# mcdiarmid/waveforms

Measured on AMD Instinct MI355X. Metric: SOQPSK-TG Msym/s mod+Viterbi-detect @8sps, higher is better.
Workload: dtype f64; 1 GPU; SOQPSK-TG 1e+07 symbols @8 sps, modulate + AWGN + PT matched filter + 4-state Viterbi detect (BASELINE configs[1]); waveform=soqpsk, sps=8, prbs=PN23, noise=Philox4x32-10 + Box-Muller (device), fuse=175, streams=1, detector_warmup_rows=16, detector_form=lanes (one chunk per lane), parallelism=independent trial blocks x1

## Files before the change

waveforms_amd/_hip.py:

```python
from __future__ import annotations

import ctypes
import threading
from ctypes import POINTER, c_char_p, c_double, c_int, c_int64, c_uint64, c_void_p
from pathlib import Path

import numpy as np

import os

_LIB_PATH = Path(os.environ.get("WF_HIP_LIBRARY") or Path(__file__).resolve().parent / "csrc" / "libwfhip.so")

WF_ERR_VALUE, WF_ERR_KEY, WF_ERR_HIP, WF_ERR_DEVICE, WF_ERR_NOMEM = -1, -2, -3, -4, -5
WF_CPM_STATE_BYTES, WF_CPM_STREAM_STATE_BYTES = 16384, 20480
(WF_OPT_CPM_FORM, WF_OPT_CPM_CHUNK_CALLS, WF_OPT_DET_REPAIR, WF_OPT_DET_FINAL_VERIFY, WF_OPT_ITERATION_SERVER,
 WF_OPT_MCB_TAIL_PERMILLE, WF_OPT_PIPE_RESERVE_CUS, WF_OPT_CPM_SAMPLES_MIN_CALLS, WF_OPT_SOFT_CHUNK_CALLS,
 WF_OPT_CPM_SOFT_CHUNK_CALLS) = range(10)

_P = c_void_p
SIGNATURES = {
    "wf_version": (c_char_p, []),
    "wf_last_error_string": (c_char_p, []),
    "wf_ctx_create": (c_int, [c_int, POINTER(c_void_p)]),
    "wf_ctx_destroy": (c_int, [_P]),
# ... 133 lines not shown
        ("warmup", c_int), ("fuse", c_int), ("event_slot", c_int), ("d_mf_factor", c_void_p),
    ]


_lib = None
_lock = threading.RLock()
_ctxs: dict[int, int] = {}


def lib() -> ctypes.CDLL:
    global _lib
    if _lib is None:
        with _lock:
            if _lib is None:
                if not _LIB_PATH.exists():
                    raise RuntimeError(
                        f"{_LIB_PATH} is missing - build it with `python -m waveforms_amd.csrc.build` "
                        "(there is no CPU fallback)")
                import torch

                handle = ctypes.CDLL(str(_LIB_PATH))
                for name, (res, args) in SIGNATURES.items():
                    fn = getattr(handle, name)
                    fn.restype, fn.argtypes = res, args
                _lib = handle
    return _lib


def torch():
    import torch as _t

    return _t


def require_device() -> int:
    t = torch()
    if not t.cuda.is_available():
        raise RuntimeError("waveforms_amd needs a HIP device (MI355X); none is visible and there is "
                           "no CPU fallback")
    return t.cuda.current_device()


def check(rc: int) -> None:
    if rc == 0:
        return
    msg = lib().wf_last_error_string().decode(errors="replace")
    if rc == WF_ERR_VALUE:
        raise ValueError(msg)
    if rc == WF_ERR_KEY:
        raise KeyError(msg)
    raise RuntimeError(f"libwfhip error {rc}: {msg}")


default_options: dict[int, int] = {}


def set_option(handle, key: int, value: int) -> None:
    check(lib().wf_ctx_set_option(handle, int(key), int(value)))


def get_option(handle, key: int) -> int:
    v = c_int64(0)
    check(lib().wf_ctx_get_option(handle, int(key), ctypes.byref(v)))
    return int(v.value)


def set_default_option(key: int, value: int) -> None:
    with _lock:
        if int(value) == 0:
            default_options.pop(int(key), None)
        else:
            default_options[int(key)] = int(value)
        for handle in _ctxs.values():
            set_option(handle, key, value)


def apply_option_args(pairs) -> None:
    for kv in pairs or []:
        key, _, val = str(kv).partition("=")
        set_default_option(globals()["WF_OPT_" + key.strip().upper()], int(val))


def ctx() -> int:
    dev = require_device()
    if dev not in _ctxs:
        with _lock:
            if dev not in _ctxs:
                out = c_void_p()
                check(lib().wf_ctx_create(dev, ctypes.byref(out)))
                for k, v in default_options.items():
                    set_option(out.value, k, v)
                if not _ctxs:
                    import atexit

                    atexit.register(_destroy_default_contexts)
                _ctxs[dev] = out.value
    return _ctxs[dev]


def _destroy_default_contexts() -> None:
    for handle in list(_ctxs.values()):
        try:
            if _lib is not None:
                _lib.wf_ctx_retire(handle)
        except Exception:
            pass


def new_ctx() -> int:
    out = c_void_p()
    check(lib().wf_ctx_create(require_device(), ctypes.byref(out)))
    for k, v in default_options.items():
        set_option(out.value, k, v)
    return out.value


def free_ctx(handle) -> None:
    if handle and _lib is not None:
        try:
            _lib.wf_ctx_destroy(handle)
        except Exception:
            pass


def stream() -> int:
    return torch().cuda.current_stream().cuda_stream


def device_check() -> None:
    check(lib().wf_ctx_check(ctx(), stream()))


_NP2T = {"uint8": "uint8", "int8": "int8", "float64": "float64", "int64": "int64", "int32": "int32", "float32": "float32"}
# ... 35 lines not shown
```

waveforms_amd/csrc/wf_common.h:

```cpp
#pragma once
#include <hip/hip_runtime.h>
#include <stdint.h>

#include <atomic>
#include <map>
#include <mutex>
#include <vector>
#include <string>

#include "../../include/wfhip.h"

#define WF_WAVE 64

void wf_set_error(const char *fmt, ...);

#define WF_HIP(call)                                                                     \
    do {                                                                                 \
        hipError_t e_ = (call);                                                          \
        if (e_ != hipSuccess) {                                                          \
            wf_set_error("%s failed: %s (%s:%d)", #call, hipGetErrorString(e_), __FILE__, \
                         __LINE__);                                                      \
            return WF_ERR_HIP;                                                           \
        }                                                                                \
    } while (0)

#define WF_REQUIRE(cond, ...)          \
    do {                               \
        if (!(cond)) {                 \
            wf_set_error(__VA_ARGS__); \
            return WF_ERR_VALUE;       \
        }                              \
    } while (0)

#define WF_LAUNCH_CHECK() WF_HIP(hipGetLastError())

enum { WF_FAULT_SCAN_TIMEOUT = 1u, WF_FAULT_LIVE_TABLE = 2u };

struct wf_lfsr_tables {
    uint64_t host[64][64];
    uint64_t *dev = nullptr;
    uint64_t f_even = 0, f_odd = 0, f_m2 = 0, f_m1 = 0;
    bool f_ready = false;
};

struct wf_ctx {
    int device = 0;
    int cus = 256;
    int64_t opt[WF_OPT_COUNT] = {0};
    uint64_t *d_scan = nullptr;
    size_t scan_words = 0;
    unsigned *d_fault = nullptr;
    unsigned *h_fault = nullptr;
    uint8_t *d_tables = nullptr;
    uint8_t h_tables_cache[2048] = {0};
    int tables_cached = 0;
    hipEvent_t tables_event = nullptr;
    hipStream_t tables_stream = nullptr;
    bool tables_pending = false;
    uint64_t *d_fsm_scratch = nullptr;
    size_t fsm_scratch_words = 0;
    int *h_small = nullptr;
    int *d_small = nullptr;
    std::map<uint64_t, wf_lfsr_tables *> lfsr;
    double *d_mod_scratch = nullptr;
    size_t mod_scratch_words = 0;
    double *d_vit_edge = nullptr;
    size_t vit_edge_words = 0;
    unsigned long long *d_vit_unmerged = nullptr;
    hipEvent_t *events = nullptr;
    void *pipe_stream = nullptr;
    void *pipe_stream2 = nullptr;
    void *pipe_pro = nullptr, *pipe_main = nullptr;
    hipEvent_t pipe_call = nullptr, pipe_pro_done = nullptr;
    hipEvent_t pipe_front = nullptr, pipe_done[2] = {nullptr, nullptr};
    bool pipe_done_valid[2] = {false, false};
    int pipe_set = 0;
    std::map<uint64_t, uint32_t> promises;
    std::mutex promises_lock;
    double *h_iter = nullptr;
    double *d_iter = nullptr;
    void *h_mailbox = nullptr;
    void *d_mailbox = nullptr;
    void *iter_stream = nullptr;
    const void *iter_last_state = nullptr;
    std::atomic_flag iter_lock = ATOMIC_FLAG_INIT;
    bool iter_closing = false;
};

static inline hipStream_t wf_stream(void *s) { return reinterpret_cast<hipStream_t>(s); }

int wf_ctx_reserve_scan(wf_ctx *ctx, size_t words);
int wf_ctx_reserve_fsm(wf_ctx *ctx, size_t words);
int wf_ctx_reserve_mod(wf_ctx *ctx, size_t words);
int wf_iter_server_stop(wf_ctx *ctx);
int wf_ctx_reserve_vit(wf_ctx *ctx, size_t words);

struct lfsr_emit_args;
int wf_lfsr_generate_dyn(wf_ctx *ctx, int degree, uint64_t mask, uint64_t state, uint64_t skip,
                         const uint64_t *d_dyn_skip, uint8_t *d_bits, int64_t n, uint64_t *h_state_out, void *stream,
                         const struct lfsr_emit_args *emit = nullptr);
int wf_lfsr_generate_map(wf_ctx *ctx, int degree, uint64_t mask, uint64_t state, uint64_t skip, uint8_t *d_bits, int64_t nbits,
                         int map_kind, int8_t *d_symbols, void *stream);
int wf_soqpsk_prbs_encode(wf_ctx *ctx, int degree, uint64_t mask, uint64_t state, uint64_t skip, const uint8_t *h_next,
                          const int8_t *h_out, uint8_t *d_bits, int64_t n, int8_t *d_symbols, void *stream, void *mid_event = nullptr);
int wf_awgn_mf_bank_dyn(wf_ctx *ctx, const double *d_signal_ri, int64_t nsamp, double rot_re, double rot_im,
                        double sigma, uint64_t seed, uint64_t stream_id, uint64_t first_index,
                        const uint64_t *d_dyn_index, const double *d_taps_ri, int nfilt, int ntaps, int64_t first,
                        int step, int64_t ncols, double *d_out_ri, void *stream, int pack_par0 = -1);
int wf_viterbi4_detect_packed(wf_ctx *ctx, const double *d_rows4, int64_t ncalls, int differential, int warmup,
                              uint8_t *d_bits, int8_t *d_syms, double *d_state, void *stream);
int wf_cpm_modulate_window(wf_ctx *ctx, const int8_t *d_symbols, int64_t sym_origin, int64_t nloc, int64_t nsym_total,
                           const double *d_h, int nh, const double *d_pulse, int ntaps, int sps, double phi0,
                           int64_t tile_lo, int64_t ntiles, double *d_out_ri, int64_t out_origin,
                           const uint64_t *d_q_in, uint64_t *d_q_out, int64_t q_out_tile, void *stream);
struct wf_mcb_opts {
    const double *pam_factor = nullptr;
    bool cpm_paired = false;
    int runs_hint = 0;
    int scratch_slot = -1;
};
int wf_mod_chan_bank_packed(wf_ctx *ctx, const int8_t *d_symbols, int64_t nsym, const double *d_h, int nh,
                            const double *d_pulse, int ntaps, int sps, double phi0, const double *d_mf_taps, double rot_re,
                            double rot_im, double sigma, uint64_t seed, uint64_t stream_id, uint64_t first_index,
                            int64_t first, int64_t ncols, int pack_par0, double *d_rows4, void *stream, int mf_ntaps = 0,
                            const wf_mcb_opts *opts = nullptr, int stage = 3);
int wf_mod_chan_bank_window(wf_ctx *ctx, const int8_t *d_symbols, int64_t sym_origin, int64_t nloc, int64_t nsym_total,
// ... 404 lines not shown
```

waveforms_amd/csrc/wf_ctx.hip:

```cpp
#include <stdarg.h>
#include <stdio.h>

#include "wf_common.h"

static thread_local char g_err[512] = "";

void wf_set_error(const char *fmt, ...)
{
    va_list ap;
    va_start(ap, fmt);
    vsnprintf(g_err, sizeof(g_err), fmt, ap);
    va_end(ap);
}

extern "C" const char *wf_version(void) { return "waveforms-amd 0.1.0 (gfx950)"; }
extern "C" const char *wf_last_error_string(void) { return g_err; }

extern "C" int wf_ctx_create(int device, wf_ctx **out)
{
    WF_REQUIRE(out != nullptr, "wf_ctx_create: out is NULL");
    int ndev = 0;
    WF_HIP(hipGetDeviceCount(&ndev));
    WF_REQUIRE(device >= 0 && device < ndev, "wf_ctx_create: device %d of %d", device, ndev);
    WF_HIP(hipSetDevice(device));
    wf_ctx *c = new wf_ctx();
    c->device = device;
    (void)hipDeviceGetAttribute(&c->cus, hipDeviceAttributeMultiprocessorCount, device);
    if (c->cus < 1) c->cus = 256;
    WF_HIP(hipMalloc(&c->d_fault, 64));
    WF_HIP(hipMemset(c->d_fault, 0, 64));
    WF_HIP(hipHostMalloc(&c->h_fault, 64, hipHostMallocDefault));
    WF_HIP(hipMalloc(&c->d_tables, 4096));
    WF_HIP(hipMalloc(&c->d_vit_unmerged, 4 * sizeof(unsigned long long)));
    WF_HIP(hipMemset(c->d_vit_unmerged, 0, 4 * sizeof(unsigned long long)));
    WF_HIP(hipMalloc(&c->d_small, 256));
    WF_HIP(hipHostMalloc(&c->h_small, 256, hipHostMallocDefault));
    *out = c;
    int rc = wf_ctx_reserve_scan(c, 1 << 16);
    if (rc) return rc;
    return wf_ctx_reserve_fsm(c, 1 << 16);
}

extern "C" int wf_ctx_destroy(wf_ctx *c)
{
    if (!c) return WF_OK;
    (void)hipSetDevice(c->device);
    (void)wf_iter_server_stop(c);
    (void)hipDeviceSynchronize();
    for (auto &kv : c->lfsr) {
        if (kv.second->dev) (void)hipFree(kv.second->dev);
        delete kv.second;
    }
    if (c->events) {
        for (int k = 0; k < WF_LINK_EVENT_SLOTS * (WF_LINK_STAGES + 1); ++k) (void)hipEventDestroy(c->events[k]);
        delete[] c->events;
    }
    if (c->pipe_front) (void)hipEventDestroy(c->pipe_front);
    for (int k = 0; k < 2; ++k)
        if (c->pipe_done[k]) (void)hipEventDestroy(c->pipe_done[k]);
    if (c->pipe_stream) (void)hipStreamDestroy(static_cast<hipStream_t>(c->pipe_stream));
    if (c->pipe_stream2) (void)hipStreamDestroy(static_cast<hipStream_t>(c->pipe_stream2));
    if (c->pipe_pro) (void)hipStreamDestroy(static_cast<hipStream_t>(c->pipe_pro));
    if (c->pipe_main) (void)hipStreamDestroy(static_cast<hipStream_t>(c->pipe_main));
    if (c->pipe_call) (void)hipEventDestroy(c->pipe_call);
    if (c->pipe_pro_done) (void)hipEventDestroy(c->pipe_pro_done);
    if (c->d_scan) (void)hipFree(c->d_scan);
    if (c->d_fsm_scratch) (void)hipFree(c->d_fsm_scratch);
    if (c->d_mod_scratch) (void)hipFree(c->d_mod_scratch);
    if (c->d_vit_edge) (void)hipFree(c->d_vit_edge);
    if (c->d_vit_unmerged) (void)hipFree(c->d_vit_unmerged);
    if (c->d_fault) (void)hipFree(c->d_fault);
    if (c->h_fault) (void)hipHostFree(c->h_fault);
    if (c->d_tables) (void)hipFree(c->d_tables);
    if (c->tables_event) (void)hipEventDestroy(c->tables_event);
    if (c->d_small) (void)hipFree(c->d_small);
    if (c->h_small) (void)hipHostFree(c->h_small);
    if (c->h_iter) (void)hipHostFree(c->h_iter);
    if (c->iter_stream) (void)hipStreamDestroy(static_cast<hipStream_t>(c->iter_stream));
    if (c->h_mailbox) (void)hipHostFree(c->h_mailbox);
    delete c;
    return WF_OK;
}

extern "C" int wf_ctx_retire(wf_ctx *c)
{
    if (!c) return WF_OK;
    (void)hipSetDevice(c->device);
    (void)wf_iter_server_stop(c);
    if (c->pipe_stream) (void)hipStreamSynchronize(static_cast<hipStream_t>(c->pipe_stream));
    if (c->pipe_stream2) (void)hipStreamSynchronize(static_cast<hipStream_t>(c->pipe_stream2));
    if (c->pipe_pro) (void)hipStreamSynchronize(static_cast<hipStream_t>(c->pipe_pro));
    if (c->pipe_main) (void)hipStreamSynchronize(static_cast<hipStream_t>(c->pipe_main));
    return WF_OK;
}

int wf_link_join_internal(wf_ctx *c, void *stream)
{
    if (!c) return WF_OK;
    for (int k = 0; k < 2; ++k)
        if (c->pipe_done_valid[k]) WF_HIP(hipStreamWaitEvent(wf_stream(stream), c->pipe_done[k], 0));
    return WF_OK;
}

extern "C" int wf_link_join(wf_ctx *c, void *stream)
{
    WF_REQUIRE(c != nullptr, "wf_link_join: ctx is NULL");
    return wf_link_join_internal(c, stream);
}

extern "C" int wf_ctx_set_option(wf_ctx *c, int key, int64_t value)
{
    WF_REQUIRE(c != nullptr, "wf_ctx_set_option: ctx is NULL");
    WF_REQUIRE(key >= 0 && key < WF_OPT_COUNT, "wf_ctx_set_option: unknown option %d", key);
    bool ok = true;
    switch (key) {
    case WF_OPT_CPM_FORM: ok = value >= 0 && value <= 2; break;
    case WF_OPT_CPM_CHUNK_CALLS: ok = value >= 0 && value <= 8192; break;
    case WF_OPT_DET_REPAIR: case WF_OPT_DET_FINAL_VERIFY: case WF_OPT_ITERATION_SERVER: ok = value == 0 || value == 1; break;
// ... 143 lines not shown
```

waveforms_amd/csrc/wf_link.h:

```cpp
#pragma once
#include "wf_common.h"

static inline int64_t round_up(int64_t v, int64_t a) { return (v + a - 1) / a * a; }

static inline int link_pipe_open(wf_ctx *ctx, const char *fn, int64_t set_bytes, int64_t workspace_bytes, bool second)
{
    WF_REQUIRE(2 * set_bytes <= workspace_bytes, "%s: fuse bit 5 needs two sets of intermediates (%lld bytes)", fn, (long long)(2 * set_bytes));
    WF_HIP(hipSetDevice(ctx->device));
    hipStream_t ps;
    if (!ctx->pipe_stream) {
        WF_HIP(hipStreamCreateWithFlags(&ps, hipStreamNonBlocking));
        ctx->pipe_stream = ps;
        WF_HIP(hipEventCreateWithFlags(&ctx->pipe_front, hipEventDisableTiming));
        for (int k = 0; k < 2; ++k) WF_HIP(hipEventCreateWithFlags(&ctx->pipe_done[k], hipEventDisableTiming));
    }
    if (second && !ctx->pipe_stream2) {
        WF_HIP(hipStreamCreateWithFlags(&ps, hipStreamNonBlocking));
        ctx->pipe_stream2 = ps;
    }
    return WF_OK;
}

static inline int link_pipe_select(wf_ctx *ctx, int64_t set_bytes, char *&w, void *waiter)
{
    w += (int64_t)ctx->pipe_set * set_bytes;
    if (ctx->pipe_done_valid[ctx->pipe_set]) WF_HIP(hipStreamWaitEvent(wf_stream(waiter), ctx->pipe_done[ctx->pipe_set], 0));
    return WF_OK;
}

static inline int link_pipe_close(wf_ctx *ctx, void *back)
{
    WF_HIP(hipEventRecord(ctx->pipe_done[ctx->pipe_set], wf_stream(back)));
    ctx->pipe_done_valid[ctx->pipe_set] = true;
    ctx->pipe_set ^= 1;
    return WF_OK;
}

static inline int link_stage_events(wf_ctx *ctx, const char *fn, int event_slot, hipEvent_t *&ev)
{
    ev = nullptr;
    if (event_slot < 0) return WF_OK;
    WF_REQUIRE(event_slot < WF_LINK_EVENT_SLOTS, "%s: event_slot %d", fn, event_slot);
    if (!ctx->events) {
        ctx->events = new hipEvent_t[WF_LINK_EVENT_SLOTS * (WF_LINK_STAGES + 1)];
        for (int k = 0; k < WF_LINK_EVENT_SLOTS * (WF_LINK_STAGES + 1); ++k) WF_HIP(hipEventCreate(&ctx->events[k]));
    }
    ev = ctx->events + event_slot * (WF_LINK_STAGES + 1);
    return WF_OK;
}

static inline int mark(hipEvent_t *ev, int k, void *stream)
{
    if (ev) WF_HIP(hipEventRecord(ev[k], wf_stream(stream)));
    return WF_OK;
}

struct link_chunk_window {
    int64_t k_lo, ncols, ws, nloc, tile_lo, tile_hi, ntiles, q_out_tile;
};

static inline link_chunk_window link_chunk_window_of(int64_t B, int64_t c, int64_t halo, int64_t N, int64_t ncalls_total, int64_t spt, int64_t ntiles_total)
{
    link_chunk_window W;
    W.k_lo = c * B;
    const int64_t k_hi = W.k_lo + B < ncalls_total ? W.k_lo + B : ncalls_total;
    W.ncols = k_hi > W.k_lo ? k_hi - W.k_lo : 0;
    W.ws = c * B - halo > 0 ? c * B - halo : 0;
    const int64_t we = (c + 1) * B + halo < N ? (c + 1) * B + halo : N;
    W.nloc = we > W.ws ? we - W.ws : 0;
    W.tile_lo = spt > 0 && c * B / spt - 1 > 0 ? c * B / spt - 1 : 0;
    W.tile_hi = spt > 0 ? (c + 1) * B / spt + 1 : 0;
    if (W.tile_hi > ntiles_total) W.tile_hi = ntiles_total;
    W.ntiles = W.tile_hi > W.tile_lo ? W.tile_hi - W.tile_lo : 0;
    const int64_t next_tile_lo = spt > 0 ? (c + 1) * B / spt - 1 : 0;
    W.q_out_tile = (next_tile_lo >= W.tile_lo && next_tile_lo < W.tile_hi) ? next_tile_lo - W.tile_lo : -1;
    return W;
}
// ... 19 lines not shown
```

waveforms_amd/csrc/wf_pipeline.hip:

```cpp
#include "wf_link.h"

__global__ void time_axis_kernel(int64_t n, double step, double *__restrict__ out)
{
    const int64_t stride = (int64_t)gridDim.x * blockDim.x;
    for (int64_t k = (int64_t)blockIdx.x * blockDim.x + threadIdx.x; k < n; k += stride)
        out[k] = (double)k * step;
}

extern "C" int wf_time_axis_f64(wf_ctx *ctx, int64_t n, double step, double *d_out, void *stream)
{
    WF_REQUIRE(ctx && n >= 0, "wf_time_axis_f64: bad argument");
    if (n == 0) return WF_OK;
    WF_REQUIRE(d_out != nullptr, "wf_time_axis_f64: NULL output");
    WF_HIP(hipSetDevice(ctx->device));
    hipLaunchKernelGGL(time_axis_kernel, dim3(wf_grid_for(n, 256, 4096)), dim3(256), 0, wf_stream(stream), n,
                       step, d_out);
    WF_LAUNCH_CHECK();
    return WF_OK;
}

struct link_layout {
    int64_t nsym, npts, ncols, first;
    size_t off_bits, off_syms, off_freq, off_sig, off_mf, off_dbits, off_dsyms, total;
};
// ... 59 lines not shown
}
static int link_check_factor(wf_ctx *ctx, const wf_link_config *cfg, void *stream)
{
    if (!cfg->d_mf_factor || cfg->mf_ntaps == cfg->sps + 1 || cfg->mf_nfilt != 3 || cfg->mf_ntaps < 1) return WF_OK;
    const int nt = cfg->mf_ntaps;
    const void *ptrs[2] = {cfg->d_mf_taps, cfg->d_mf_factor};
    const size_t nb[2] = {(size_t)3 * nt * 16, (size_t)(2 * nt + 12) * 8};
    return wf_promise_verified(ctx, 2, ptrs, nb, 2, stream, link_factor_matches, &nt,
                               "wf_link_config.d_mf_factor does not reproduce d_mf_taps (taps[s] != sum_k G[s][k] b_k to 1e-12)");
}

extern "C" int64_t wf_link_workspace_bytes(const wf_link_config *cfg)
{
    if (!cfg || cfg->nsym < 1 || cfg->sps < 1) return -1;
    const int64_t one = (int64_t)make_layout(cfg->nsym, cfg->sps, cfg->ntaps, cfg->mf_nfilt, 2, cfg->timing_offset).total;
    return link_pipelined(cfg) ? 2 * round_up(one, 256) : one;
}

static hipStream_t link_masked_stream(const wf_ctx *ctx, int reserve)
{
    hipStream_t s = nullptr;
    if (reserve > 0 && reserve < ctx->cus) {
        const int words = (ctx->cus + 31) / 32;
        std::vector<uint32_t> mask((size_t)words, 0u);
        for (int cu = reserve; cu < ctx->cus; ++cu) mask[(size_t)(cu / 32)] |= 1u << (cu % 32);
        if (hipExtStreamCreateWithCUMask(&s, (uint32_t)words, mask.data()) == hipSuccess) return s;
        (void)hipGetLastError();
        s = nullptr;
    }
    if (hipStreamCreateWithFlags(&s, hipStreamDefault) != hipSuccess) return nullptr;
    return s;
}

extern "C" int wf_link_run(wf_ctx *ctx, const wf_link_config *cfg, void *d_workspace, int64_t workspace_bytes,
                           int64_t *d_counts, int64_t *h_compared, void *stream)
{
    WF_REQUIRE(ctx && cfg && d_workspace && d_counts, "wf_link_run: NULL argument");
    WF_REQUIRE(cfg->nsym >= 1 && cfg->sps >= 1 && cfg->mf_nfilt == 3, "wf_link_run: bad configuration");
    WF_REQUIRE((reinterpret_cast<uintptr_t>(d_workspace) & 255) == 0, "wf_link_run: workspace must be 256-byte aligned");
    const int length = 2;
    const link_layout L = make_layout(cfg->nsym, cfg->sps, cfg->ntaps, cfg->mf_nfilt, length, cfg->timing_offset);
    WF_REQUIRE((int64_t)L.total <= workspace_bytes, "wf_link_run: workspace too small (%lld < %lld)",
               (long long)workspace_bytes, (long long)L.total);
    WF_REQUIRE(L.npts >= cfg->mf_ntaps, "wf_link_run: burst shorter than the matched filter");
    char *w = static_cast<char *>(d_workspace);
    const bool piped = link_pipelined(cfg) && L.ncols > 0;
    void *s_pro = stream, *s_main = stream;
    bool ahead = false;
    int slot = -1, rc;
    if (piped) {
        const int64_t set_bytes = round_up((int64_t)L.total, 256);
        if ((rc = link_pipe_open(ctx, "wf_link_run", set_bytes, workspace_bytes, false))) return rc;
        const int64_t rsv = ctx->opt[WF_OPT_PIPE_RESERVE_CUS];
        ahead = rsv != 0;
        if (ahead) {
            if (!ctx->pipe_pro) {
                hipStream_t sp;
                WF_HIP(hipStreamCreateWithFlags(&sp, hipStreamDefault));
                ctx->pipe_pro = sp;
                ctx->pipe_main = link_masked_stream(ctx, rsv < 0 ? 0 : (int)rsv);
                WF_REQUIRE(ctx->pipe_main != nullptr, "wf_link_run: could not create the front end's stream");
                WF_HIP(hipEventCreateWithFlags(&ctx->pipe_call, hipEventDisableTiming));
                WF_HIP(hipEventCreateWithFlags(&ctx->pipe_pro_done, hipEventDisableTiming));
            }
            s_pro = ctx->pipe_pro;
            s_main = ctx->pipe_main;
            slot = ctx->pipe_set;
            if (stream) {
                WF_HIP(hipEventRecord(ctx->pipe_call, wf_stream(stream)));
                WF_HIP(hipStreamWaitEvent(wf_stream(s_pro), ctx->pipe_call, 0));
            }
        }
        if ((rc = link_pipe_select(ctx, set_bytes, w, s_pro))) return rc;
    } else if ((rc = wf_link_join_internal(ctx, stream))) {
        return rc;
    }
    uint8_t *bits = reinterpret_cast<uint8_t *>(w + L.off_bits);
    int8_t *syms = reinterpret_cast<int8_t *>(w + L.off_syms);
    double *freq = reinterpret_cast<double *>(w + L.off_freq);
    double *sig = reinterpret_cast<double *>(w + L.off_sig);
    double *mf = reinterpret_cast<double *>(w + L.off_mf);
    uint8_t *dbits = reinterpret_cast<uint8_t *>(w + L.off_dbits);
    int8_t *dsyms = reinterpret_cast<int8_t *>(w + L.off_dsyms);

    const soqpsk_trellis_tables T = soqpsk_trellis(cfg->differential);
    hipEvent_t *ev;
    if ((rc = link_stage_events(ctx, "wf_link_run", cfg->event_slot, ev))) return rc;
    if ((rc = mark(ev, 0, s_pro))) return rc;
    rc = (cfg->fuse & 16) ? 1 : wf_soqpsk_prbs_encode(ctx, cfg->degree, cfg->mask, cfg->state, cfg->skip, &T.next[0][0][0], &T.outp[0][0][0], bits,
                                                       cfg->nsym, syms, s_pro, ev ? (void *)ev[1] : nullptr);
    if (rc < 0) return rc;
    if (rc == 1) {
        if ((rc = wf_lfsr_generate(ctx, cfg->degree, cfg->mask, cfg->state, cfg->skip, bits, cfg->nsym, nullptr, s_pro))) return rc;
        if ((rc = mark(ev, 1, s_pro))) return rc;
        if ((rc = wf_fsm_encode(ctx, &T.next[0][0][0], &T.outp[0][0][0], 2, 4, 1, bits, cfg->nsym, 0, 0, syms, nullptr, s_pro))) return rc;
    }
    if (!ahead && (rc = mark(ev, 2, s_pro))) return rc;
    bool fused_all = false;
    if (link_one_kernel(cfg) && L.ncols > 0) {
        wf_mcb_opts mo;
        mo.pam_factor = cfg->d_mf_factor;
        mo.scratch_slot = slot;
        if ((rc = link_check_factor(ctx, cfg, stream))) return rc;
        for (int stage = ahead ? 1 : 3; stage <= (ahead ? 2 : 3); ++stage) {
            if (ahead && stage == 2) {
                if ((rc = mark(ev, 2, s_pro))) return rc;
                WF_HIP(hipEventRecord(ctx->pipe_pro_done, wf_stream(s_pro)));
                WF_HIP(hipStreamWaitEvent(wf_stream(s_main), ctx->pipe_pro_done, 0));
                if ((rc = mark(ev, 3, s_main))) return rc;
            }
            rc = wf_mod_chan_bank_packed(ctx, syms, cfg->nsym, cfg->d_h, 1, cfg->d_pulse, cfg->ntaps, cfg->sps, M_PI / 4, cfg->d_mf_taps,
                                         cos(-M_PI / 4), sin(-M_PI / 4), cfg->sigma, cfg->seed, cfg->stream_id, 0, L.first, L.ncols, 0,
                                         mf, stage == 1 ? s_pro : s_main, cfg->mf_ntaps, &mo, stage);
            if (rc < 0) return rc;
            WF_REQUIRE(rc == 0, "wf_link_run: internal: the one-kernel front end refused a configuration wf_mod_chan_bank_applies accepted");
        }
        fused_all = true;
    }
    if (fused_all) {
        if (!ahead && (rc = mark(ev, 3, s_main))) return rc;
        if ((rc = mark(ev, 4, s_main)) || (rc = mark(ev, 5, s_main))) return rc;
        void *back = stream;
        if (piped) {
            back = ctx->pipe_stream;
            WF_HIP(hipEventRecord(ctx->pipe_front, wf_stream(s_main)));
            WF_HIP(hipStreamWaitEvent(wf_stream(back), ctx->pipe_front, 0));
        }
        if ((rc = mark(ev, 6, back))) return rc;
        rc = wf_viterbi4_detect_packed(ctx, mf, L.ncols, cfg->differential, link_warmup(cfg), dbits, dsyms, nullptr, back);
        if (rc) return rc;
        if ((rc = mark(ev, 7, back))) return rc;
        int64_t m_ = L.ncols - length;
        if (m_ > cfg->nsym) m_ = cfg->nsym;
        if (m_ < 0) m_ = 0;
        if ((rc = wf_count_errors(ctx, dsyms + length, syms, dbits + length, bits, m_, d_counts, back))) return rc;
        if ((rc = mark(ev, 8, back))) return rc;
        if (piped && (rc = link_pipe_close(ctx, back))) return rc;
        if (h_compared) *h_compared = m_;
        return WF_OK;
    }
    bool fused_mod = false;
    if (cfg->fuse & 1) {
        rc = wf_cpm_modulate_c128(ctx, syms, cfg->nsym, cfg->d_h, 1, cfg->d_pulse, cfg->ntaps, cfg->sps, M_PI / 4, sig, stream);
        if (rc < 0) return rc;
        fused_mod = rc == 0;
    }
    if (fused_mod) {
        if ((rc = mark(ev, 3, stream))) return rc;
    } else {
        if ((rc = wf_upsample_fir_f64(ctx, syms, cfg->nsym, cfg->d_h, 1, cfg->d_pulse, cfg->ntaps, cfg->sps, freq, stream))) return rc;
        if ((rc = mark(ev, 3, stream))) return rc;
        if ((rc = wf_phase_cexp_f64(ctx, freq, L.npts, cfg->sps, M_PI / 4, 0.0, sig, nullptr, stream))) return rc;
    }
    if ((rc = mark(ev, 4, stream))) return rc;
    const double rot_re = cos(-M_PI / 4), rot_im = sin(-M_PI / 4);
    const bool fused_chan = (cfg->fuse & 2) && L.ncols > 0;
    if (!fused_chan)
        if ((rc = wf_awgn_c128(ctx, sig, L.npts, rot_re, rot_im, cfg->sigma, cfg->seed, cfg->stream_id, 0, sig, stream))) return rc;
    if ((rc = mark(ev, 5, stream))) return rc;
    int64_t m = L.ncols - length;
    if (m > cfg->nsym) m = cfg->nsym;
    if (m < 0) m = 0;
    const bool packed = fused_chan && link_packed_rows8(cfg);
    if (L.ncols > 0) {
        if (packed)
            rc = wf_awgn_mf_bank_dyn(ctx, sig, L.npts, rot_re, rot_im, cfg->sigma, cfg->seed, cfg->stream_id, 0, nullptr,
                                     cfg->d_mf_taps, cfg->mf_nfilt, cfg->mf_ntaps, L.first, cfg->sps, L.ncols, mf, stream, 0);
        else if (fused_chan)
            rc = wf_awgn_mf_bank_c128(ctx, sig, L.npts, rot_re, rot_im, cfg->sigma, cfg->seed, cfg->stream_id, 0,
                                      cfg->d_mf_taps, cfg->mf_nfilt, cfg->mf_ntaps, L.first, cfg->sps, L.ncols, mf, stream);
        else
            rc = wf_mf_bank_c128(ctx, sig, L.npts, cfg->d_mf_taps, cfg->mf_nfilt, cfg->mf_ntaps, L.first, cfg->sps,
                                 L.ncols, mf, stream);
        if (rc) return rc;
        if ((rc = mark(ev, 6, stream))) return rc;
        if (packed)
            rc = wf_viterbi4_detect_packed(ctx, mf, L.ncols, cfg->differential, link_warmup(cfg), dbits, dsyms, nullptr, stream);
        else
            rc = wf_viterbi4_detect(ctx, mf, L.ncols, cfg->differential, link_warmup(cfg), dbits, dsyms, nullptr, stream);
// ... 251 lines not shown
```

waveforms_amd/csrc/wf_viterbi.hip:

```cpp
#include <stddef.h>
#include <stdlib.h>
#include <string.h>

#include <time.h>

#include "wf_viterbi4.h"

#define VIT_THREADS 256
#define VIT_DEFAULT_WARMUP 31
#define VIT_MAX_LEN 64

template <int COL>
__device__ __forceinline__ void vit_acs(const double m[4], const vit_comp &q, double out[4], uint64_t second[4])
{
    double fa[4], fb[4];
    if (COL == 0) {
        fa[0] = m[0] - q.i1; fb[0] = m[2] + q.a;
        fa[1] = m[1] - q.r1; fb[1] = m[3] + q.b;
        fa[2] = m[0] - q.b;  fb[2] = m[2] + q.r1;
        fa[3] = m[1] - q.a;  fb[3] = m[3] + q.i1;
    } else {
        fa[0] = m[0] - q.i1; fb[0] = m[1] - q.b;
        fa[1] = m[0] - q.a;  fb[1] = m[1] - q.r1;
        fa[2] = m[2] + q.r1; fb[2] = m[3] + q.a;
// ... 20 lines not shown
{
    constexpr int PREV = COL ^ 1;
    const vit_comp now = vit_components<COL, PACKED>(zrow);
    const double mn = fmin(fmin(L.m0[0], L.m0[1]), fmin(L.m0[2], L.m0[3]));
    const double carried[4] = {L.m0[0] - mn, L.m0[1] - mn, L.m0[2] - mn, L.m0[3] - mn};
    double ma[4], mb[4];
    uint64_t n0[4], n1[4];
    vit_acs<PREV>(carried, L.prev, ma, n0);
    vit_acs<COL>(ma, now, mb, n1);
    const uint64_t c01 = __builtin_amdgcn_ballot_w64(mb[1] < mb[0]), c23 = __builtin_amdgcn_ballot_w64(mb[3] < mb[2]);
    const double v01 = fmin(mb[0], mb[1]), v23 = fmin(mb[2], mb[3]);
    const uint64_t s1b1 = __builtin_amdgcn_ballot_w64(v23 < v01);
    const uint64_t s1b0 = vit_mux(s1b1, c23, c01);
    const uint64_t w1 = vit_mux(s1b1, vit_mux(c23, n1[3], n1[2]), vit_mux(c01, n1[1], n1[0]));
    const uint64_t e0b0 = COL == 0 ? s1b0 : w1;
    const uint64_t e0b1 = COL == 0 ? w1 : s1b1;
    const uint64_t w0 = vit_mux(e0b1, vit_mux(e0b0, n0[3], n0[2]), vit_mux(e0b0, n0[1], n0[0]));
    const uint64_t st0b0 = PREV == 0 ? e0b0 : w0;
    const uint64_t st0b1 = PREV == 0 ? w0 : e0b1;
    const uint64_t b0 = PREV == 0 ? e0b1 : e0b0, b1 = st0b0, b2 = st0b1;
    const uint64_t bit_m = b0 ^ (diff ? (PREV == 0 ? st0b1 : st0b0) : 0ull);
    const uint64_t x02 = b0 ^ b2, x01 = b0 ^ b1, x12 = b1 ^ b2;
    const uint64_t cd0_m = PREV == 0 ? ~x02 : ~x01;
    const uint64_t cd1_m = PREV == 0 ? (x02 & ~x12) : (x01 & ~x02);
    bit = __builtin_amdgcn_inverse_ballot_w64(bit_m);
    cd0 = __builtin_amdgcn_inverse_ballot_w64(cd0_m);
    cd1 = __builtin_amdgcn_inverse_ballot_w64(cd1_m);
#pragma unroll
    for (int s = 0; s < 4; ++s) L.m0[s] = ma[s];
    L.prev = now;
}

template <int COL, bool PACKED>
__device__ __forceinline__ void vit_step(vit_lane &L, const double2 *__restrict__ zrow, bool prime, int diff,
                                         int64_t k, int64_t a, int64_t ncalls, uint64_t *__restrict__ dec)
{
    if (prime) {
        L.prev = vit_components<COL, PACKED>(zrow);
        return;
    }
    bool bit, cd0, cd1;
    vit_step_core<COL, PACKED>(L, zrow, diff, bit, cd0, cd1);
    if (k >= a) {
        const int c = (int)(k - a) & 15;
        L.wb |= (bit ? 1u : 0u) << c;
        L.ws |= ((cd0 ? 1u : 0u) | (cd1 ? 2u : 0u)) << (2 * c);
        if (c == 15 || k + 1 == ncalls) {
            dec[(int)(k - a) >> 4] = (uint64_t)L.wb | ((uint64_t)L.ws << 32);
            L.wb = L.ws = 0;
        }
    }
}

__device__ __forceinline__ uint64_t vit_spread_bits8(uint32_t x)
{
    const uint64_t t = ((uint64_t)(x & 0xFF) * 0x0101010101010101ull) & 0x8040201008040201ull;
    return ((t + 0x7F7F7F7F7F7F7F7Full) >> 7) & 0x0101010101010101ull;
}

__device__ __forceinline__ uint64_t vit_spread_syms8(uint32_t x)
{
    uint64_t t = ((uint64_t)(x & 0xFFFF) | ((uint64_t)(x & 0xFFFF) << 24)) & 0x000000FF000000FFull;
    t = (t | (t << 12)) & 0x000F000F000F000Full;
    t = (t | (t << 6)) & 0x0303030303030303ull;
    const uint64_t v = t << 1;
    return ((v & 0x7F7F7F7F7F7F7F7Full) + 0x7E7E7E7E7E7E7E7Eull) ^ ((v ^ 0xFEFEFEFEFEFEFEFEull) & 0x8080808080808080ull);
}

__device__ __forceinline__ void vit_flush(const uint64_t *__restrict__ dec, int ch, int64_t a, int64_t ncalls,
                                          uint8_t *__restrict__ bits, int8_t *__restrict__ syms)
{
    for (int gq = 0; gq < ch / 16; ++gq) {
        const int64_t k0 = a + 16 * gq;
        if (k0 >= ncalls) break;
        const uint64_t w = dec[gq];
        const uint32_t wb = (uint32_t)w, ws = (uint32_t)(w >> 32);
        const uint64_t b_lo = vit_spread_bits8(wb), b_hi = vit_spread_bits8(wb >> 8);
        const uint64_t s_lo = vit_spread_syms8(ws), s_hi = vit_spread_syms8(ws >> 16);
        if (k0 + 16 <= ncalls) {
            *reinterpret_cast<ulonglong2 *>(bits + k0) = make_ulonglong2(b_lo, b_hi);
            *reinterpret_cast<ulonglong2 *>(syms + k0) = make_ulonglong2(s_lo, s_hi);
        } else {
            for (int q = 0; k0 + q < ncalls; ++q) {
                bits[k0 + q] = (uint8_t)(((q < 8 ? b_lo : b_hi) >> (8 * (q & 7))) & 0xFF);
                syms[k0 + q] = (int8_t)(((q < 8 ? s_lo : s_hi) >> (8 * (q & 7))) & 0xFF);
            }
        }
    }
}

__device__ __forceinline__ void vit_save_start(vit_lane &L)
{
#pragma unroll
    for (int s4 = 0; s4 < 4; ++s4) L.ms[s4] = L.m0[s4];
}

__device__ __forceinline__ vit_comp vit_comp_from_inc(const double *inc, int col)
{
    vit_comp c;
    c.i1 = inc[7];
    if (col == 0) { c.a = inc[4]; c.r1 = inc[5]; c.b = inc[6]; }
    else { c.r1 = inc[4]; c.b = inc[5]; c.a = inc[6]; }
    return c;
}

__device__ __forceinline__ void vit_comp_to_inc(const vit_comp &c, int col, double *inc)
{
    if (col == 0) {
        inc[0] = -c.i1; inc[1] = -c.b; inc[2] = -c.r1; inc[3] = -c.a;
        inc[4] = c.a;   inc[5] = c.r1; inc[6] = c.b;   inc[7] = c.i1;
    } else {
        inc[0] = -c.i1; inc[1] = -c.a; inc[2] = -c.b;  inc[3] = -c.r1;
        inc[4] = c.r1;  inc[5] = c.b;  inc[6] = c.a;   inc[7] = c.i1;
    }
}

#define VIT_S 4
#ifndef VIT_DEPTH
#define VIT_DEPTH 3
#endif
#define VIT_PIECES_RW(RW) ((RW) * VIT_S)
#define VIT_PIECES (3 * VIT_S)
#define VIT_LANE_SLOTS (VIT_PIECES + 1)

__device__ __forceinline__ double2 vit_ld16(const double2 *p)
{
    typedef double v2d __attribute__((ext_vector_type(2)));
    const v2d v = __builtin_nontemporal_load(reinterpret_cast<const v2d *>(p));
    return make_double2(v.x, v.y);
}

template <int PAR0, bool PACKED>
__device__ __forceinline__ void viterbi_batch_body(const double *__restrict__ mf, int64_t ncalls, int CH, int diff, int warmup,
                                                   uint8_t *__restrict__ bits, int8_t *__restrict__ syms,
                                                   double *__restrict__ state, int64_t i0, double2 (*s_rows)[WF_WAVE * VIT_LANE_SLOTS],
                                                   uint64_t *__restrict__ s_dec, double *__restrict__ edge)
{
    constexpr int RW = PACKED ? 2 : 3;
    constexpr int NP = VIT_PIECES_RW(RW);
    constexpr int LS = NP + 1;
    const int lane = threadIdx.x & 63, wave = threadIdx.x >> 6;
    const int64_t g0 = ((int64_t)blockIdx.x * (VIT_THREADS / WF_WAVE) + wave) * WF_WAVE;
    const int64_t a = (g0 + lane) * CH;
    const bool live = a < ncalls;
    const int nsteps = warmup + 1 + CH;
    const int nbatch = (nsteps + VIT_S - 1) / VIT_S;
    const double2 *rows = reinterpret_cast<const double2 *>(mf);
    double2 *tile = s_rows[wave];
    uint64_t *dec = s_dec + (wave * WF_WAVE + lane) * (CH / 16 + 1);
// ... 2 lines not shown
#pragma unroll
    for (int u = 0; u < NP; ++u) {
        const int p = u * WF_WAVE + lane;
        const int sg = p / NP;
        sgw[u] = (sg << 8) | (p - sg * NP);
    }
    const int64_t g0u = __builtin_amdgcn_readfirstlane((int)(g0 >> 6)) * (int64_t)WF_WAVE;
    auto fetch = [&](int b, double2 dst[NP]) __attribute__((always_inline)) {
        const int64_t rb = g0u * CH - warmup - 1 + (int64_t)b * VIT_S;
        const double2 *basep = rows + RW * rb;
        if (rb >= 0 && rb + (int64_t)(WF_WAVE - 1) * CH + VIT_S <= ncalls) {
#pragma unroll
            for (int u = 0; u < NP; ++u) dst[u] = vit_ld16(basep + RW * CH * (sgw[u] >> 8) + (sgw[u] & 255));
        } else {
            const int64_t lo64 = -rb, hi64 = ncalls - 1 - rb;
            const int lo = lo64 < -(1 << 30) ? -(1 << 30) : (lo64 > (1 << 30) ? (1 << 30) : (int)lo64);
            const int hi = hi64 < -(1 << 30) ? -(1 << 30) : (hi64 > (1 << 30) ? (1 << 30) : (int)hi64);
#pragma unroll
            for (int u = 0; u < NP; ++u) {
                const int sg = sgw[u] >> 8, wi = sgw[u] & 255;
                const int rrel = sg * CH + wi / RW;
                const int rc = min(max(rrel, lo), hi);
                dst[u] = vit_ld16(basep + RW * rc + (wi - RW * (wi / RW)));
            }
        }
    };
    auto stash = [&](const double2 src[NP]) __attribute__((always_inline)) {
#pragma unroll
        for (int u = 0; u < NP; ++u) tile[(sgw[u] >> 8) * LS + (sgw[u] & 255)] = src[u];
    };

    vit_lane L;
#pragma unroll
    for (int k = 0; k < 4; ++k) L.m0[k] = 0.0;
    L.prev.r1 = L.prev.i1 = L.prev.a = L.prev.b = 0.0;
    L.wb = L.ws = 0;
    if (state && a == 0) {
#pragma unroll
        for (int k = 0; k < 4; ++k) L.m0[k] = state[1 + k];
        L.prev = vit_comp_from_inc(state + 5, (int)((i0 - 1) & 1));
    }
#if VIT_DEPTH == 3
    double2 pend0[NP], pend1[NP], pend2[NP];
#else
    double2 pend0[NP], pend1[NP];
#endif
    const int last_b = nbatch - 1;
    fetch(0, pend0);
    fetch(min(1, last_b), pend1);
#if VIT_DEPTH == 3
    fetch(min(2, last_b), pend2);
#endif
    const int64_t kbase = a - warmup - 1;
    auto round = [&](int b, double2 (&pd)[NP]) __attribute__((always_inline)) {
        stash(pd);
        fetch(min(b + VIT_DEPTH, last_b), pd);
        __builtin_amdgcn_fence(__ATOMIC_RELEASE, "wavefront");
        __builtin_amdgcn_wave_barrier();
        __builtin_amdgcn_fence(__ATOMIC_ACQUIRE, "wavefront");
        if (live) {
#pragma unroll 1
            for (int jj = 0; jj < VIT_S; jj += 2) {
                const int j = b * VIT_S + jj;
                const int64_t k = kbase + j;
                const double2 *zr = tile + lane * LS + RW * jj;
                if (j == warmup + 1) vit_save_start(L);
                if (j < nsteps && k >= 0 && k < ncalls)
                    vit_step<PAR0, PACKED>(L, zr, j == 0, diff, k, a, ncalls, dec);
                if (j + 1 == warmup + 1) vit_save_start(L);
                if (j + 1 < nsteps && k + 1 >= 0 && k + 1 < ncalls)
                    vit_step<PAR0 ^ 1, PACKED>(L, zr + RW, false, diff, k + 1, a, ncalls, dec);
            }
        }
        __builtin_amdgcn_fence(__ATOMIC_RELEASE, "wavefront");
        __builtin_amdgcn_wave_barrier();
        __builtin_amdgcn_fence(__ATOMIC_ACQUIRE, "wavefront");
    };
    for (int b0 = 0; b0 < nbatch; b0 += VIT_DEPTH) {
        round(b0, pend0);
        round(b0 + 1, pend1);
#if VIT_DEPTH == 3
        round(b0 + 2, pend2);
#endif
    }
    if (live) vit_flush(dec, CH, a, ncalls, bits, syms);
    if (edge && live) {
        double *e = edge + 8 * (g0 + lane);
        *reinterpret_cast<double4 *>(e) = make_double4(L.ms[0], L.ms[1], L.ms[2], L.ms[3]);
        *reinterpret_cast<double4 *>(e + 4) = make_double4(L.m0[0], L.m0[1], L.m0[2], L.m0[3]);
    }
    if (state && live && a + CH >= ncalls) {
        state[16] = (double)(i0 + ncalls);
#pragma unroll
        for (int k = 0; k < 4; ++k) state[17 + k] = L.m0[k];
        vit_comp_to_inc(L.prev, (int)((i0 + ncalls - 1) & 1), state + 21);
    }
}

#ifndef VIT_MIN_WAVES
#define VIT_MIN_WAVES 1
#endif
template <bool PACKED>
__global__ __launch_bounds__(VIT_THREADS, VIT_MIN_WAVES) void viterbi_batch_kernel(const double *__restrict__ mf, int64_t ncalls,
                                                                     int ch, int diff, int warmup, uint8_t *__restrict__ bits,
                                                                     int8_t *__restrict__ syms, double *__restrict__ state,
                                                                     double *__restrict__ edge, int64_t nchunks)
{
    __shared__ double2 s_rows[VIT_THREADS / WF_WAVE][WF_WAVE * VIT_LANE_SLOTS];
    extern __shared__ uint64_t s_dec[];
    const int64_t i0 = state ? (int64_t)state[0] : 0;
    if (blockIdx.x == 0 && threadIdx.x < VIT_HDR) reinterpret_cast<uint64_t *>(edge + 8 * nchunks)[threadIdx.x] = 0;
    if ((i0 - warmup - 1) & 1) viterbi_batch_body<1, PACKED>(mf, ncalls, ch, diff, warmup, bits, syms, state, i0, s_rows, s_dec, edge);
    else viterbi_batch_body<0, PACKED>(mf, ncalls, ch, diff, warmup, bits, syms, state, i0, s_rows, s_dec, edge);
// ... 960 lines not shown
```

waveforms_amd/link.py:

```python
from __future__ import annotations

import ctypes
import math

import numpy as np

from . import _hip
from .cpm.soqpsk import freq_pulse_soqpsk_tg
from .filters.matched import pack_bank_factors, pam_bank_factors, pam_matched_filter_taps, pt_matched_filter_taps
from .glfsr.pn import generate_mask


def sigma_for_ebn0(ebn0_db: float, sps: int) -> float:
    return math.sqrt(sps / (2.0 * 10.0 ** (ebn0_db / 10.0)))


def operating_point_warmup(waveform: str, ebn0_db: float | None) -> int:
    if ebn0_db is None:
        return 0
    if waveform == "soqpsk":
        return 16 if ebn0_db >= 6.0 else 0
    if waveform == "multih":
        return 48 if ebn0_db >= 8.0 else (64 if ebn0_db >= 6.0 else 0)
    return 64 if ebn0_db >= 3.0 else 0
# ... 148 lines not shown
            if getattr(self, "cfg", None) is not None and (self.cfg.fuse & 32) and getattr(self, "workspace", None) is not None:
                _hip.lib().wf_link_join(self._ctx, _hip.stream())
                _hip.torch().cuda.current_stream().synchronize()
        except Exception:
            pass
        self._close()

    def layout(self) -> dict:
        return self._words(self.LAYOUT, self.LAYOUT_KEYS)

    def reset_counts(self) -> None:
        _hip.check(_hip.lib().wf_link_join(self._ctx, _hip.stream()))
        self.counts.zero_()
        self.compared = 0

    def stage_ms(self, event_slot: int) -> dict[str, float]:
        buf = (ctypes.c_float * len(self.STAGES))()
        _hip.check(_hip.lib().wf_link_stage_ms(self._ctx, event_slot, buf))
        return {k: float(v) for k, v in zip(self.STAGES, buf) if k != "-"}

    def launch(self, counts_ptr: int, ebn0_db: float | None, seed: int, stream_id: int, skip_bits: int, event_slot: int = -1,
               warmup: int | None = None) -> int:
        c = self.cfg
        c.sigma, c.seed, c.stream_id, c.skip, c.event_slot = self._sigma(ebn0_db), seed, stream_id, skip_bits, event_slot
        keep = c.warmup
        if warmup is not None:
            c.warmup = warmup
        m = ctypes.c_int64(0)
        try:
            _hip.check(getattr(_hip.lib(), self.RUN)(self._ctx, ctypes.byref(c), self.workspace.data_ptr(), self.workspace_bytes,
                                                     counts_ptr, ctypes.byref(m), _hip.stream()))
        finally:
            c.warmup = keep
        return m.value

    def run_block(self, ebn0_db: float | None, seed: int = 1, stream_id: int = 0, skip_bits: int = 0, event_slot: int = -1) -> None:
        self.compared += self.launch(self.counts.data_ptr(), ebn0_db, seed, stream_id, skip_bits, event_slot)


class SOQPSKLink(_SOQPSK, _Link):

    @property
    def row_bytes(self) -> int:
        return self.layout()["row_bytes"]

    def stage_ms(self, event_slot: int) -> dict[str, float]:
        d = super().stage_ms(event_slot)
        if self.prologue_ahead:
            d["fir"], d["phase"] = d["phase"], 0.0
        return d

    @property
    def prologue_ahead(self) -> bool:
        return bool(self.cfg.fuse & 32) and bool(self.layout()["one_kernel_front_end"]) and _hip.get_option(self._ctx, _hip.WF_OPT_PIPE_RESERVE_CUS) != 0


class CPMLink(_CPM, _Link):
    """Device-resident link for the waveforms served by the generic CPM trellis detector
    (``wf_cpm_link_run``): PRBS -> mapper -> cpm_modulate -> AWGN -> matched-filter rows ->
    detector -> error count."""


class _Stream(_Session):

    WAITS = ()
    _ctx2 = None

    def __init__(self, total_symbols: int, chunk_symbols: int, sps: int = 8, **kw) -> None:
        self._configure(int(total_symbols), sps, **kw)
        self.total_symbols, self.chunk_symbols = int(total_symbols), int(chunk_symbols)
        lib = _hip.lib()
        nbytes = getattr(lib, self.STREAM_WORKSPACE_BYTES)(ctypes.byref(self.cfg), self.chunk_symbols)
        if nbytes < 0:
            tl, spt, nt = ctypes.c_int64(), ctypes.c_int64(), ctypes.c_int64()
            lib.wf_mod_tile_geometry(self.sps, self.cfg.ntaps, self.total_symbols, ctypes.byref(tl), ctypes.byref(spt), ctypes.byref(nt))
            raise ValueError(self._chunk_rule(spt.value))
        self._allocate(nbytes)
        self.state = self._carry()
        self.total_calls = self._total_calls()
        self.nchunks = -(-self.total_calls // self.chunk_symbols)

    def __del__(self):
        if self._ctx2:
            _hip.free_ctx(self._ctx2)
            self._ctx2 = None
        self._close()

    def reset(self) -> None:
        self.state.zero_()
        self.counts.zero_()
        self.compared = 0

    def chunk_info(self, c: int) -> dict:
        return self._words(self.STREAM_LAYOUT, self.CHUNK_KEYS, self.chunk_symbols, c)

    def _point(self, ebn0_db: float | None, seed: int, stream_id: int):
        cfg = self.cfg
        cfg.sigma, cfg.seed, cfg.stream_id, cfg.event_slot = self._sigma(ebn0_db), seed, stream_id, -1
        return cfg

    def run_chunk(self, c: int, ebn0_db: float | None, seed: int = 1, stream_id: int = 0) -> None:
        m = ctypes.c_int64(0)
        _hip.check(getattr(_hip.lib(), self.STREAM_CHUNK)(self._ctx, ctypes.byref(self._point(ebn0_db, seed, stream_id)), self.chunk_symbols, c,
                                                          self.state.data_ptr(), self.workspace.data_ptr(), self.workspace_bytes,
                                                          self.counts.data_ptr(), ctypes.byref(m), _hip.stream()))
        self.compared += m.value

# ... 169 lines not shown
```

Baseline: 21770 Msym/s.

## Enable prologue-ahead pipelining by default and add interior fast path in Viterbi

Makes the pipe-reserve-CUs option default to -1, which enables the prologue-ahead front end whenever the matched filter has sps+1 taps. The prologue then runs on the caller's stream, the front-end stream waits on the previous back-end start, and front-end ordering is tracked across mode switches. Separately, the Viterbi kernel gains an interior path for wavefronts whose chunks lie entirely inside the call range, which skips the per-step bounds checks on k. The changes aim to overlap the front end with the detector and to cut branch overhead in the hot loop. In exchange they add cross-stream dependencies and a second inner-loop variant.

```diff
diff --git a/waveforms_amd/_hip.py b/waveforms_amd/_hip.py
--- a/waveforms_amd/_hip.py
+++ b/waveforms_amd/_hip.py
@@ -209,6 +209,7 @@
     raise RuntimeError(f"libwfhip error {rc}: {msg}")
 
 
+LIBRARY_DEFAULT_OPTIONS = {WF_OPT_PIPE_RESERVE_CUS: -1}
 default_options: dict[int, int] = {}
 
 
@@ -222,9 +223,11 @@
     return int(v.value)
 
 
-def set_default_option(key: int, value: int) -> None:
+def set_default_option(key: int, value: int, literal: bool = False) -> None:
     with _lock:
-        if int(value) == 0:
+        if int(value) == 0 and not literal:
+            value = LIBRARY_DEFAULT_OPTIONS.get(int(key), 0)
+        if int(value) == LIBRARY_DEFAULT_OPTIONS.get(int(key), 0):
             default_options.pop(int(key), None)
         else:
             default_options[int(key)] = int(value)
@@ -235,7 +238,7 @@
 def apply_option_args(pairs) -> None:
     for kv in pairs or []:
         key, _, val = str(kv).partition("=")
-        set_default_option(globals()["WF_OPT_" + key.strip().upper()], int(val))
+        set_default_option(globals()["WF_OPT_" + key.strip().upper()], int(val), literal=True)
 
 
 def ctx() -> int:
diff --git a/waveforms_amd/csrc/wf_common.h b/waveforms_amd/csrc/wf_common.h
--- a/waveforms_amd/csrc/wf_common.h
+++ b/waveforms_amd/csrc/wf_common.h
@@ -71,7 +71,11 @@
     void *pipe_stream = nullptr;
     void *pipe_stream2 = nullptr;
     void *pipe_pro = nullptr, *pipe_main = nullptr;
-    hipEvent_t pipe_call = nullptr, pipe_pro_done = nullptr;
+    hipEvent_t pipe_pro_done = nullptr;
+    hipEvent_t pipe_back_go = nullptr;
+    bool pipe_back_go_valid = false;
+    bool pipe_front_recorded = false;
+    bool pipe_front_on_main = false;
     hipEvent_t pipe_front = nullptr, pipe_done[2] = {nullptr, nullptr};
     bool pipe_done_valid[2] = {false, false};
     int pipe_set = 0;
diff --git a/waveforms_amd/csrc/wf_ctx.hip b/waveforms_amd/csrc/wf_ctx.hip
--- a/waveforms_amd/csrc/wf_ctx.hip
+++ b/waveforms_amd/csrc/wf_ctx.hip
@@ -27,6 +27,7 @@
     c->device = device;
     (void)hipDeviceGetAttribute(&c->cus, hipDeviceAttributeMultiprocessorCount, device);
     if (c->cus < 1) c->cus = 256;
+    c->opt[WF_OPT_PIPE_RESERVE_CUS] = -1;
     WF_HIP(hipMalloc(&c->d_fault, 64));
     WF_HIP(hipMemset(c->d_fault, 0, 64));
     WF_HIP(hipHostMalloc(&c->h_fault, 64, hipHostMallocDefault));
@@ -62,8 +63,8 @@
     if (c->pipe_stream2) (void)hipStreamDestroy(static_cast<hipStream_t>(c->pipe_stream2));
     if (c->pipe_pro) (void)hipStreamDestroy(static_cast<hipStream_t>(c->pipe_pro));
     if (c->pipe_main) (void)hipStreamDestroy(static_cast<hipStream_t>(c->pipe_main));
-    if (c->pipe_call) (void)hipEventDestroy(c->pipe_call);
     if (c->pipe_pro_done) (void)hipEventDestroy(c->pipe_pro_done);
+    if (c->pipe_back_go) (void)hipEventDestroy(c->pipe_back_go);
     if (c->d_scan) (void)hipFree(c->d_scan);
     if (c->d_fsm_scratch) (void)hipFree(c->d_fsm_scratch);
     if (c->d_mod_scratch) (void)hipFree(c->d_mod_scratch);
diff --git a/waveforms_amd/csrc/wf_link.h b/waveforms_amd/csrc/wf_link.h
--- a/waveforms_amd/csrc/wf_link.h
+++ b/waveforms_amd/csrc/wf_link.h
@@ -21,8 +21,11 @@
     return WF_OK;
 }
 
-static inline int link_pipe_select(wf_ctx *ctx, int64_t set_bytes, char *&w, void *waiter)
+static inline int link_pipe_select(wf_ctx *ctx, int64_t set_bytes, char *&w, void *waiter, bool on_main = false)
 {
+    if (ctx->pipe_front_on_main != on_main && ctx->pipe_front_recorded) WF_HIP(hipStreamWaitEvent(wf_stream(waiter), ctx->pipe_front, 0));
+    ctx->pipe_front_on_main = on_main;
+    ctx->pipe_front_recorded = true;
     w += (int64_t)ctx->pipe_set * set_bytes;
     if (ctx->pipe_done_valid[ctx->pipe_set]) WF_HIP(hipStreamWaitEvent(wf_stream(waiter), ctx->pipe_done[ctx->pipe_set], 0));
     return WF_OK;
diff --git a/waveforms_amd/csrc/wf_pipeline.hip b/waveforms_amd/csrc/wf_pipeline.hip
--- a/waveforms_amd/csrc/wf_pipeline.hip
+++ b/waveforms_amd/csrc/wf_pipeline.hip
@@ -135,26 +135,24 @@
         const int64_t set_bytes = round_up((int64_t)L.total, 256);
         if ((rc = link_pipe_open(ctx, "wf_link_run", set_bytes, workspace_bytes, false))) return rc;
         const int64_t rsv = ctx->opt[WF_OPT_PIPE_RESERVE_CUS];
-        ahead = rsv != 0;
+        ahead = rsv > 0 || (rsv < 0 && cfg->mf_ntaps == cfg->sps + 1);
         if (ahead) {
             if (!ctx->pipe_pro) {
                 hipStream_t sp;
                 WF_HIP(hipStreamCreateWithFlags(&sp, hipStreamDefault));
                 ctx->pipe_pro = sp;
+            }
+            if (!ctx->pipe_main) {
                 ctx->pipe_main = link_masked_stream(ctx, rsv < 0 ? 0 : (int)rsv);
                 WF_REQUIRE(ctx->pipe_main != nullptr, "wf_link_run: could not create the front end's stream");
-                WF_HIP(hipEventCreateWithFlags(&ctx->pipe_call, hipEventDisableTiming));
-                WF_HIP(hipEventCreateWithFlags(&ctx->pipe_pro_done, hipEventDisableTiming));
             }
-            s_pro = ctx->pipe_pro;
+            if (!ctx->pipe_pro_done) WF_HIP(hipEventCreateWithFlags(&ctx->pipe_pro_done, hipEventDisableTiming));
+            if (!ctx->pipe_back_go) WF_HIP(hipEventCreateWithFlags(&ctx->pipe_back_go, hipEventDisableTiming));
+            s_pro = stream ? stream : ctx->pipe_pro;
             s_main = ctx->pipe_main;
             slot = ctx->pipe_set;
-            if (stream) {
-                WF_HIP(hipEventRecord(ctx->pipe_call, wf_stream(stream)));
-                WF_HIP(hipStreamWaitEvent(wf_stream(s_pro), ctx->pipe_call, 0));
-            }
         }
-        if ((rc = link_pipe_select(ctx, set_bytes, w, s_pro))) return rc;
+        if ((rc = link_pipe_select(ctx, set_bytes, w, s_pro, ahead))) return rc;
     } else if ((rc = wf_link_join_internal(ctx, stream))) {
         return rc;
     }
@@ -190,6 +188,7 @@
                 if ((rc = mark(ev, 2, s_pro))) return rc;
                 WF_HIP(hipEventRecord(ctx->pipe_pro_done, wf_stream(s_pro)));
                 WF_HIP(hipStreamWaitEvent(wf_stream(s_main), ctx->pipe_pro_done, 0));
+                if (ctx->pipe_back_go_valid) WF_HIP(hipStreamWaitEvent(wf_stream(s_main), ctx->pipe_back_go, 0));
                 if ((rc = mark(ev, 3, s_main))) return rc;
             }
             rc = wf_mod_chan_bank_packed(ctx, syms, cfg->nsym, cfg->d_h, 1, cfg->d_pulse, cfg->ntaps, cfg->sps, M_PI / 4, cfg->d_mf_taps,
@@ -208,6 +207,10 @@
             back = ctx->pipe_stream;
             WF_HIP(hipEventRecord(ctx->pipe_front, wf_stream(s_main)));
             WF_HIP(hipStreamWaitEvent(wf_stream(back), ctx->pipe_front, 0));
+            if (ahead) {
+                WF_HIP(hipEventRecord(ctx->pipe_back_go, wf_stream(back)));
+                ctx->pipe_back_go_valid = true;
+            }
         }
         if ((rc = mark(ev, 6, back))) return rc;
         rc = wf_viterbi4_detect_packed(ctx, mf, L.ncols, cfg->differential, link_warmup(cfg), dbits, dsyms, nullptr, back);
diff --git a/waveforms_amd/csrc/wf_viterbi.hip b/waveforms_amd/csrc/wf_viterbi.hip
--- a/waveforms_amd/csrc/wf_viterbi.hip
+++ b/waveforms_amd/csrc/wf_viterbi.hip
@@ -96,6 +96,35 @@
     }
 }
 
+__device__ __forceinline__ void vit_save_start(vit_lane &L)
+{
+#pragma unroll
+    for (int s4 = 0; s4 < 4; ++s4) L.ms[s4] = L.m0[s4];
+}
+
+template <int COL, bool PACKED>
+__device__ __forceinline__ void vit_step_interior(vit_lane &L, const double2 *__restrict__ zrow, int diff, int j, int warmup, int nsteps,
+                                                  uint64_t *__restrict__ dec)
+{
+    if (j >= nsteps) return;
+    if (j == 0) {
+        L.prev = vit_components<COL, PACKED>(zrow);
+        return;
+    }
+    if (j == warmup + 1) vit_save_start(L);
+    bool bit, cd0, cd1;
+    vit_step_core<COL, PACKED>(L, zrow, diff, bit, cd0, cd1);
+    if (j > warmup) {
+        const int o = j - warmup - 1, c = o & 15;
+        L.wb |= (bit ? 1u : 0u) << c;
+        L.ws |= ((cd0 ? 1u : 0u) << (2 * c)) | ((cd1 ? 2u : 0u) << (2 * c));
+        if (c == 15) {
+            dec[o >> 4] = (uint64_t)L.wb | ((uint64_t)L.ws << 32);
+            L.wb = L.ws = 0;
+        }
+    }
+}
+
 __device__ __forceinline__ uint64_t vit_spread_bits8(uint32_t x)
 {
     const uint64_t t = ((uint64_t)(x & 0xFF) * 0x0101010101010101ull) & 0x8040201008040201ull;
@@ -133,12 +162,6 @@
     }
 }
 
-__device__ __forceinline__ void vit_save_start(vit_lane &L)
-{
-#pragma unroll
-    for (int s4 = 0; s4 < 4; ++s4) L.ms[s4] = L.m0[s4];
-}
-
 __device__ __forceinline__ vit_comp vit_comp_from_inc(const double *inc, int col)
 {
     vit_comp c;
@@ -247,13 +270,22 @@
     fetch(min(2, last_b), pend2);
 #endif
     const int64_t kbase = a - warmup - 1;
+    const bool interior = g0u * CH - warmup - 1 >= 0 && (g0u + WF_WAVE) * CH <= ncalls;
     auto round = [&](int b, double2 (&pd)[NP]) __attribute__((always_inline)) {
         stash(pd);
         fetch(min(b + VIT_DEPTH, last_b), pd);
         __builtin_amdgcn_fence(__ATOMIC_RELEASE, "wavefront");
         __builtin_amdgcn_wave_barrier();
         __builtin_amdgcn_fence(__ATOMIC_ACQUIRE, "wavefront");
-        if (live) {
+        if (interior) {
+#pragma unroll 1
+            for (int jj = 0; jj < VIT_S; jj += 2) {
+                const int j = b * VIT_S + jj;
+                const double2 *zr = tile + lane * LS + RW * jj;
+                vit_step_interior<PAR0, PACKED>(L, zr, diff, j, warmup, nsteps, dec);
+                vit_step_interior<PAR0 ^ 1, PACKED>(L, zr + RW, diff, j + 1, warmup, nsteps, dec);
+            }
+        } else if (live) {
 #pragma unroll 1
             for (int jj = 0; jj < VIT_S; jj += 2) {
                 const int j = b * VIT_S + jj;
diff --git a/waveforms_amd/link.py b/waveforms_amd/link.py
--- a/waveforms_amd/link.py
+++ b/waveforms_amd/link.py
@@ -224,7 +224,9 @@
 
     @property
     def prologue_ahead(self) -> bool:
-        return bool(self.cfg.fuse & 32) and bool(self.layout()["one_kernel_front_end"]) and _hip.get_option(self._ctx, _hip.WF_OPT_PIPE_RESERVE_CUS) != 0
+        rsv = _hip.get_option(self._ctx, _hip.WF_OPT_PIPE_RESERVE_CUS)
+        ahead = rsv > 0 or (rsv < 0 and self.cfg.mf_ntaps == self.cfg.sps + 1)
+        return bool(self.cfg.fuse & 32) and bool(self.layout()["one_kernel_front_end"]) and ahead
 
 
 class CPMLink(_CPM, _Link):
```

After: 22940 Msym/s (median of 6 runs). 5.4% higher.
